# Borda/pyImSegm

Hardware: NVIDIA H100
Metric: megapixels/sec end-to-end SLIC+features+GC (pipe_color2d_slic_features_model_graphcut) (higher is better)
Workload: dtype f64

## Files before the change

include/imsegm_b200.h:

```cpp
#ifndef IMSEGM_B200_H
#define IMSEGM_B200_H

#include <stddef.h>
#include <stdint.h>

#ifdef __cplusplus
extern "C" {
#endif

typedef void* isb_stream_t;

enum isb_status {
    ISB_OK = 0,
    ISB_ERR_ARG = -1,
    ISB_ERR_CUDA = -2,
    ISB_ERR_CAPACITY = -3,
    ISB_ERR_UNSUPPORTED = -4
};

enum isb_dtype { ISB_U8 = 0, ISB_U16 = 1, ISB_F32 = 2, ISB_F64 = 3, ISB_I8 = 4, ISB_I16 = 5, ISB_I32 = 6, ISB_U32 = 7, ISB_I64 = 8, ISB_BOOL = 9 };

const char* isb_last_error(void);
int isb_abi_version(void);
long long isb_launch_count(void);
int isb_note_graph_replay(long long n_kernels);
int isb_profile_enable(int on);
int isb_profile_stage_count(void);
const char* isb_profile_stage_name(int id);
int isb_profile_collect(double* ms_out , long long* count_out );


int isb_slic_prepare(const void* img, int dtype, int H, int W, int C, const double* w_half, int radius, double ratio,
                     int rescale, double* lab_planar, double* minmax_out , isb_stream_t stream);

int isb_image_minmax(const void* img, int dtype, long long n, double* minmax_out , isb_stream_t stream);

size_t isb_slic_kmeans_workspace_bytes(int H, int W, int n_seeds, int step_y, int step_x);

int isb_slic_kmeans(const double* lab_planar, int H, int W, const double* seeds_yx, int n_seeds, int step_y, int step_x,
                    double step, int max_iter, int slic_zero, int32_t* labels, double* centroids, void* ws, size_t ws_bytes,
                    isb_stream_t stream);

int isb_slic_set_tile_cap(int cap);
long long isb_slic_full_scan_tiles(void);

typedef struct isb_slic_band {
    int32_t slab_rows, width;
    int32_t image_rows, y_off;
    int32_t own_lo, own_hi;
    int32_t halo;
    int32_t n_seeds, step_y, step_x, slic_zero;
    double step;
    const double* lab_slab;
    size_t plane_stride;
    const double* seeds_yx;
    int32_t* labels_slab;
    void* ws; size_t ws_bytes;
} isb_slic_band_t;
int isb_slic_band_begin(const isb_slic_band_t* band, isb_stream_t stream);
int isb_slic_band_assign(const isb_slic_band_t* band, isb_stream_t stream);
int isb_slic_band_update(const isb_slic_band_t* band, int64_t* xchg, isb_stream_t stream);
int isb_slic_band_import(const isb_slic_band_t* band, const int64_t* xchg, uint64_t* maxdc_xchg ,
                         isb_stream_t stream);
int isb_slic_band_finalize(const isb_slic_band_t* band, const uint64_t* maxdc_xchg, isb_stream_t stream);

size_t isb_connectivity_workspace_bytes(int H, int W);


int isb_enforce_connectivity(const int32_t* labels, int H, int W, int min_size, int max_size, int32_t* out,
                             int32_t* n_labels_out, void* ws, size_t ws_bytes, isb_stream_t stream);

int isb_slic3d_prepare(const void* vol, int dtype, int D, int H, int W, const double* w_z, int r_z, const double* w_y, int r_y,
                       const double* w_x, int r_x, double ratio, double* tmp, double* out, isb_stream_t stream);
size_t isb_slic3d_kmeans_workspace_bytes(int D, int H, int W, int n_seeds);
int isb_slic3d_kmeans(const double* vol_scaled, int D, int H, int W, const double* seeds_zyx, int n_seeds, int step_z, int step_y,
                      int step_x, double step, const double* spacing_host, int max_iter, int32_t* labels, void* ws, size_t ws_bytes,
                      isb_stream_t stream);
size_t isb_connectivity3d_workspace_bytes(int D, int H, int W, int max_size);
int isb_enforce_connectivity3d(const int32_t* labels, int D, int H, int W, int min_size, int max_size, int32_t* out,
                               int32_t* n_labels_out, void* ws, size_t ws_bytes, isb_stream_t stream);


size_t isb_segment_stats_workspace_bytes(int nb);
int isb_segment_stats_2d(const void* img, int dtype, const int32_t* seg, int H, int W, int nb, int flags, double* feat,
                         int ld, int col0, double* centres, int32_t* counts, void* ws, size_t ws_bytes, isb_stream_t stream);

int isb_segment_stats_accumulate(const void* img, int dtype, const int32_t* seg, int H, int W, int y_off, int nb, double* acc,
                                 int64_t* iacc, isb_stream_t stream);
int isb_segment_stats_deviation(const void* img, int dtype, const int32_t* seg, int H, int W, int nb, const double* acc,
                                const int64_t* iacc, float* meanf_scratch , double* var, isb_stream_t stream);
int isb_segment_stats_finish(int nb, int flags, const double* acc, const double* var, const int64_t* iacc, double* feat, int ld,
                             int col0, double* centres, int32_t* counts, isb_stream_t stream);

size_t isb_gray_stats_workspace_bytes(int nb);
int isb_gray_stats(const void* img, int dtype, const int32_t* seg, long long n, int nb, int flags, double* feat, int ld, int col0,
                   void* ws, size_t ws_bytes, isb_stream_t stream);

int isb_label_hist_2d(const int16_t* segm_select, const int16_t* struc_elem, int H, int W, int nb_labels, uint32_t* hist,
                      isb_stream_t stream);

int isb_region_label_hist(const int32_t* slic, const int32_t* annot, int H, int W, int nb_slic, int nb_annot, uint32_t* hist,
                          isb_stream_t stream);

int isb_filter_response_2d(const double* img, int n_slices, int H, int W, const double* kernels, int n_kernels, int kh, int kw,
                           double* out, isb_stream_t stream);

int isb_gaussian_filter_2d(const double* img, int n_slices, int H, int W, const double* w_half, int radius, double* tmp, double* out,
                           isb_stream_t stream);

enum isb_color_space { ISB_COLOR_HSV = 0, ISB_COLOR_LUV = 1, ISB_COLOR_LAB = 2, ISB_COLOR_HED = 3, ISB_COLOR_XYZ = 4 };
int isb_color_convert(const void* img, int dtype, long long n_px, int space, double* out, isb_stream_t stream);
int isb_gradient_sum_2d(const void* img, int dtype, int H, int W, int channels, void* out, isb_stream_t stream);
int isb_segment_median_2d(const void* img, int dtype, const int32_t* seg, int H, int W, int channels, int nb, double* feat, int ld,
                          int col0, void* ws, size_t ws_bytes, isb_stream_t stream);

int isb_lm_background(const void* img, int dtype, int H, int W, const double* w_half, int radius, const double* mix, double* planar,
                      double* tmp, double* smooth, isb_stream_t stream);
size_t isb_lm_battery_workspace_bytes(void);
int isb_lm_battery_response(const double* planar, int H, int W, const double* kernels, int n_kernels, int kh, int kw, double max_signal,
                            double* resp, double* out, void* ws, size_t ws_bytes, isb_stream_t stream);
int isb_lm_battery_partial(const double* planar, int H, int W, const double* kernels, int n_kernels, int kh, int kw, double max_signal,
                           int row_lo, int row_hi, double* resp, double* sumsq, void* ws, size_t ws_bytes, isb_stream_t stream);
int isb_lm_battery_scale(const double* resp, int H, int W, int row_lo, int row_hi, double max_signal, const double* sumsq, double* out,
                         isb_stream_t stream);

int isb_disc_label_hist(const int32_t* segm, const double* proba, int H, int W, const int32_t* positions, int n_pos,
                        const int32_t* diameters, int n_diam, const uint8_t* selem, int mh, int mw, int nb_labels, double* hist,
                        double* sizes, isb_stream_t stream);

int isb_ray_features_2d(const int8_t* seg_binary, int H, int W, const int32_t* positions, int n_pos, const float* sin_a,
                        const float* cos_a, int n_ang, int edge, float* out, isb_stream_t stream);


size_t isb_adjacency_workspace_bytes(int nb, int cap);
int isb_adjacency_edges(const int32_t* seg, int H, int W, int nb, int32_t* edges, int cap, int32_t* n_edges_out, void* ws,
                        size_t ws_bytes, isb_stream_t stream);

int isb_adjacency_edges_3d(const int32_t* seg, int D, int H, int W, int nb, int32_t* edges, int cap, int32_t* n_edges_out, void* ws,
                           size_t ws_bytes, isb_stream_t stream);
int isb_centroids_3d(const int32_t* seg, int D, int H, int W, int nb, double* centres, void* ws, size_t ws_bytes, isb_stream_t stream);

int isb_gc_energies(const double* proba, int N, const int32_t* n_nodes_dev , int K, const int32_t* edges, int E,
                    const int32_t* n_edges_dev,
                    const double* centres, int metric, int spatial, double edge_cost, const double* pairwise ,
                    double* unary, double* edge_w, int32_t* unary_i, int32_t* edge_wi, int32_t* smooth_i, void* ws,
                    size_t ws_bytes, isb_stream_t stream);
size_t isb_gc_energies_workspace_bytes(int N, int K, int E);

size_t isb_alpha_expansion_workspace_bytes(int N, int K, int E);
int isb_alpha_expansion(int N, const int32_t* n_nodes_dev , int K, int E, const int32_t* n_edges_dev,
                        const int32_t* edges, const int32_t* edge_wi,
                        const int32_t* unary_i, const int32_t* smooth_i, int n_iter, int32_t* labels, int64_t* energy_out,
                        int32_t* stats_out , void* ws, size_t ws_bytes,
                        isb_stream_t stream);

size_t isb_mixture_fit_workspace_bytes(int kind, int N, int D, int K, int n_init);
int isb_mixture_fit_params_len(int kind, int D, int K);
int isb_mixture_fit_predict(int kind, const double* feat, int N, int D, int ld, const int32_t* n_dev, int K, int n_init, int max_iter,
                            double tol, double reg_covar, int use_scaler, unsigned long long seed, const int32_t* init_labels, double* proba,
                            double* params_out, void* ws, size_t ws_bytes, isb_stream_t stream);
size_t isb_pca_workspace_bytes(int N, int D);
int isb_pca_params_len(int D);
int isb_pca_fit(const double* feat, int N, int D, int ld, const int32_t* n_dev, int use_scaler, double coef, int n_components,
                double* params_out, int32_t* n_components_out, void* ws, size_t ws_bytes, isb_stream_t stream);

size_t isb_class_transform_workspace_bytes(int N, int D_in, int has_pca);
int isb_class_transform(const double* feat, int N, int ld, const int32_t* n_dev, int D_in, const double* sc_mean, const double* sc_scale,
                        const double* pca_comp, const double* pca_mean, const double* pca_scale, int D_out, double* out, void* ws,
                        size_t ws_bytes, isb_stream_t stream);
size_t isb_mixture_predict_workspace_bytes(int N, int D, int K);
int isb_mixture_predict_proba(const double* x, int N, const int32_t* n_dev, int D, int K, const double* prec_chol, const double* bvec,
                              const double* log_const, double* proba, void* ws, size_t ws_bytes, isb_stream_t stream);
size_t isb_forest_predict_workspace_bytes(int N, int n_trees);
int isb_forest_predict_proba(const double* x, int N, const int32_t* n_dev, int D, int n_trees, const int32_t* roots, const int32_t* feature,
                             const double* threshold, const int32_t* left, const int32_t* right, int n_nodes, const double* value, int K,
                             int average, double* proba, void* ws, size_t ws_bytes, isb_stream_t stream);
size_t isb_knn_predict_workspace_bytes(int N, int N_t, int k);
int isb_knn_predict_proba(const double* x, int N, const int32_t* n_dev, int D, const double* fit_x, int N_t, const int32_t* y, int k, int K,
                          int weights, double* proba, void* ws, size_t ws_bytes, isb_stream_t stream);
size_t isb_linear_predict_workspace_bytes(int N, int n_coef);
int isb_linear_predict_proba(const double* x, int N, const int32_t* n_dev, int D, const double* coef, const double* intercept, int n_coef,
                             double* proba, void* ws, size_t ws_bytes, isb_stream_t stream);

size_t isb_lm_workspace_bytes(int H, int W, int nb, int n_batt);
int isb_lm_texture(const void* img, int dtype, const int32_t* seg, int H, int W, int nb, const double* bg_weights, int bg_radius,
                   const double* chmix_host, const float* w_tc, int NP, int orient, int n_batt, int flags,
                   double* feat, int ld, int col0, void* ws, size_t ws_bytes, isb_stream_t stream);
size_t isb_lm_acc_doubles(int nb, int n_batt);
int isb_lm_texture_accumulate(const void* img, int dtype, const int32_t* seg, int slab_rows, int W, int y_first, int y_end, int nb,
                              const double* bg_weights, int bg_radius, const double* chmix_host, const float* w_tc, int NP, int orient,
                              int n_batt, double* acc, int32_t* counts, void* ws, size_t ws_bytes, isb_stream_t stream);
int isb_lm_texture_finish(int nb, int n_batt, int flags, const double* acc, const int32_t* counts, double* feat, int ld, int col0,
                          isb_stream_t stream);

int isb_wgmma_selftest(const float* A, const float* B, int N, int K, int variant, float* D, isb_stream_t stream);

size_t isb_segment_median_workspace_bytes(long long n_px, int nb);
int isb_segment_median(const void* img, int dtype, const int32_t* seg, long long n_px, int channels, int nb, double* out, void* ws,
                       size_t ws_bytes, isb_stream_t stream);


int isb_ellipse_ransac(int T, const int32_t* trial_centre, const int32_t* samp_off, const int32_t* samp_idx, const double* params_in,
                       int C, const double* pts, const int32_t* pt_off, double thr, const double* sp_pts, const int32_t* sp_lab,
                       const double* lab_term, int N, int32_t* ok, double* params_out, int32_t* n_inl, double* crit,
                       double* resid_out, const long long* resid_off, isb_stream_t stream);
int isb_ellipse_overlap(const int32_t* segm, int H, int W, int n_labels, const int32_t* bbox_host, const double* geom_host,
                        uint8_t* mask, unsigned long long* counts, isb_stream_t stream);
int isb_binary_morph_footprint(const uint8_t* in, int H, int W, const int32_t* offsets, int n_offsets, int op, uint8_t* out,
                               isb_stream_t stream);


int isb_label_boundary_map(const int32_t* seg, int H, int W, uint8_t* out, isb_stream_t stream);
int isb_label_contour_map(const int32_t* seg, int H, int W, int32_t label, int include_boundary, uint8_t* out, isb_stream_t stream);
size_t isb_edt_workspace_bytes(int H, int W);
int isb_edt_2d(const uint8_t* sites, int H, int W, double* dist, void* ws, size_t ws_bytes, isb_stream_t stream);
size_t isb_edt_index_workspace_bytes(int H, int W);
int isb_edt_2d_indices(const uint8_t* sites, int H, int W, int32_t* index, void* ws, size_t ws_bytes, isb_stream_t stream);
size_t isb_mask_compact_workspace_bytes(int H, int W);
int isb_mask_compact_count(const uint8_t* mask, int H, int W, void* ws, size_t ws_bytes, long long* total, isb_stream_t stream);
int isb_mask_compact_write(const uint8_t* mask, int H, int W, const double* values, const void* ws, size_t ws_bytes, int64_t* points,
                           double* values_out, isb_stream_t stream);
int isb_relabel_gather(const int32_t* seg, long long npx, const int32_t* lut, int n_lut, int32_t* out, isb_stream_t stream);


int isb_color_hist(const uint8_t* img, long long n_px, int channels, int accumulate, unsigned long long* hist, isb_stream_t stream);
size_t isb_color_hist_workspace_bytes(void);
int isb_color_hist_compact_count(const unsigned long long* hist, void* ws, size_t ws_bytes, long long* total, isb_stream_t stream);
int isb_color_hist_compact_write(const unsigned long long* hist, const void* ws, size_t ws_bytes, int32_t* colors, int64_t* counts,
                                 isb_stream_t stream);
int isb_palette_map(const void* img, int dtype, long long n_px, int channels, const void* palette, int n_colors, int mode,
                    const int64_t* values, int64_t* labels, uint8_t* matched, unsigned long long* unmatched, isb_stream_t stream);
int isb_palette_gather(const int64_t* labels, long long n_px, const int64_t* keys, int n_colors, const void* table, int row_bytes,
                       void* out, unsigned long long* missing, isb_stream_t stream);
int isb_gather_at_index(const void* src, int elem_bytes, const int32_t* index, long long n, void* out, isb_stream_t stream);


size_t isb_contingency_workspace_bytes(int dtype_true, int dtype_pred);
int isb_contingency_count(const void* y_true, int dtype_true, const void* y_pred, int dtype_pred, long long n, const int64_t* drop, int n_drop,
                          void* ws, size_t ws_bytes, long long* info, isb_stream_t stream);
int isb_contingency_write(const void* y_true, int dtype_true, const void* y_pred, int dtype_pred, long long n, const int64_t* drop, int n_drop,
                          const long long* info, void* ws, size_t ws_bytes, int64_t* values_true, int64_t* values_pred, int64_t* counts,
                          isb_stream_t stream);

size_t isb_kmeans_workspace_bytes(int n, int k, int D);
int isb_kmeans_lloyd(const double* X, int n, int D, int k, int max_iter, int sweeps, double tol, double* centres, int32_t* labels, int32_t* status,
                     double* sums, int32_t* counts, double* inertia, void* ws, size_t ws_bytes, isb_stream_t stream);
int isb_kmeans_nearest(const double* X, int n, int D, const double* centres, int k, int32_t* nearest, void* ws, size_t ws_bytes,
                       isb_stream_t stream);

size_t isb_forest_fit_workspace_bytes(int n, int D, int T, int K, int max_features);
int isb_forest_fit(const float* x, int n, int D, const int32_t* y, int K, const int32_t* counts, int T, const uint64_t* seeds, int max_features,
                   int min_samples_split, int min_samples_leaf, int max_depth, double min_impurity_decrease, int cap, int32_t* left, int32_t* right,
                   int32_t* feature, double* threshold, double* impurity, int32_t* n_node_samples, double* weighted_n_node_samples,
                   uint8_t* missing_go_to_left, int32_t* class_counts, int32_t* node_count, int* n_levels , void* ws, size_t ws_bytes,
                   isb_stream_t stream);

size_t isb_forest_fit_groups_workspace_bytes(int n, int Dmax, int G, int T, int K, int max_features_max);
int isb_forest_fit_groups(const float* x, int n, int Dmax, int G, const int32_t* D , const int32_t* max_features ,
                          const int32_t* min_samples_split , const int32_t* min_samples_leaf , const int32_t* y, int K,
                          const int32_t* counts, int T, const int32_t* tree_group , const uint64_t* seeds, int max_depth,
                          double min_impurity_decrease, int cap, int32_t* left, int32_t* right, int32_t* feature, double* threshold,
                          double* impurity, int32_t* n_node_samples, double* weighted_n_node_samples, uint8_t* missing_go_to_left,
                          int32_t* class_counts, int32_t* node_count, int* n_levels , void* ws, size_t ws_bytes, isb_stream_t stream);

size_t isb_extra_trees_fit_workspace_bytes(int n, int D, int T, int K, int max_features);
int isb_extra_trees_fit(const float* x, int n, int D, const int32_t* y, int K, const int32_t* counts, int T, const uint32_t* rand_r_state,
                        int max_features, int min_samples_split, int min_samples_leaf, int max_depth, double min_impurity_decrease,
                        int small_rows, int cap, int32_t* left, int32_t* right, int32_t* feature, double* threshold, double* impurity,
                        int32_t* n_node_samples, double* weighted_n_node_samples, uint8_t* missing_go_to_left, int32_t* class_counts,
                        int32_t* node_count, void* ws, size_t ws_bytes, isb_stream_t stream);

int isb_fill_i32(int32_t* dst, long long n, int32_t value, isb_stream_t stream);

int isb_combine(void* dst, const void* src, long long n, int op, isb_stream_t stream);

int isb_gather(const int32_t* seg, long long npx, const int32_t* lut_i, const double* lut_p, int K, int32_t* out_i,
               double* out_p, isb_stream_t stream);

#ifdef __cplusplus
}
#endif
#endif
```

pyimsegm_b200/_lib.py:

```python
import ctypes as C
import os

_HERE = os.path.dirname(os.path.abspath(__file__))
LIB_PATH = os.path.join(_HERE, 'libimsegm_b200.so')

_lib = None

ISB_OK, ISB_ERR_ARG, ISB_ERR_CUDA, ISB_ERR_CAPACITY, ISB_ERR_UNSUPPORTED = 0, -1, -2, -3, -4
DTYPE_CODES = {'uint8': 0, 'uint16': 1, 'float32': 2, 'float64': 3}

_vp, _i, _d, _sz, _ll = C.c_void_p, C.c_int, C.c_double, C.c_size_t, C.c_longlong



class SlicBand(C.Structure):
    _fields_ = [('slab_rows', C.c_int32), ('width', C.c_int32), ('image_rows', C.c_int32), ('y_off', C.c_int32),
                ('own_lo', C.c_int32), ('own_hi', C.c_int32), ('halo', C.c_int32),
                ('n_seeds', C.c_int32), ('step_y', C.c_int32), ('step_x', C.c_int32), ('slic_zero', C.c_int32),
                ('step', C.c_double), ('lab_slab', C.c_void_p), ('plane_stride', C.c_size_t), ('seeds_yx', C.c_void_p),
                ('labels_slab', C.c_void_p), ('ws', C.c_void_p), ('ws_bytes', C.c_size_t)]


_bp = C.POINTER(SlicBand)

SIGNATURES = {
    'isb_last_error': (C.c_char_p, []),
    'isb_abi_version': (_i, []),
    'isb_launch_count': (_ll, []),
    'isb_note_graph_replay': (_i, [_ll]),
    'isb_profile_enable': (_i, [_i]),
    'isb_profile_stage_count': (_i, []),
    'isb_profile_stage_name': (C.c_char_p, [_i]),
    'isb_profile_collect': (_i, [C.POINTER(_d), C.POINTER(_ll)]),
    'isb_slic_prepare': (_i, [_vp, _i, _i, _i, _i, C.POINTER(_d), _i, _d, _i, _vp, _vp, _vp]),
    'isb_image_minmax': (_i, [_vp, _i, _ll, _vp, _vp]),
    'isb_slic_band_begin': (_i, [_bp, _vp]),
    'isb_slic_band_assign': (_i, [_bp, _vp]),
    'isb_slic_band_update': (_i, [_bp, _vp, _vp]),
    'isb_slic_band_import': (_i, [_bp, _vp, _vp, _vp]),
    'isb_slic_band_finalize': (_i, [_bp, _vp, _vp]),
    'isb_segment_stats_accumulate': (_i, [_vp, _i, _vp, _i, _i, _i, _i, _vp, _vp, _vp]),
    'isb_segment_stats_deviation': (_i, [_vp, _i, _vp, _i, _i, _i, _vp, _vp, _vp, _vp, _vp]),
    'isb_segment_stats_finish': (_i, [_i, _i, _vp, _vp, _vp, _vp, _i, _i, _vp, _vp, _vp]),
    'isb_slic_kmeans_workspace_bytes': (_sz, [_i, _i, _i, _i, _i]),
    'isb_slic_kmeans': (_i, [_vp, _i, _i, _vp, _i, _i, _i, _d, _i, _i, _vp, _vp, _vp, _sz, _vp]),
    'isb_slic_set_tile_cap': (_i, [_i]),
    'isb_slic_full_scan_tiles': (_ll, []),
    'isb_slic3d_prepare': (_i, [_vp, _i, _i, _i, _i, _vp, _i, _vp, _i, _vp, _i, _d, _vp, _vp, _vp]),
    'isb_slic3d_kmeans_workspace_bytes': (_sz, [_i, _i, _i, _i]),
    'isb_slic3d_kmeans': (_i, [_vp, _i, _i, _i, _vp, _i, _i, _i, _i, _d, C.POINTER(_d), _i, _vp, _vp, _sz, _vp]),
    'isb_connectivity3d_workspace_bytes': (_sz, [_i, _i, _i, _i]),
    'isb_enforce_connectivity3d': (_i, [_vp, _i, _i, _i, _i, _i, _vp, _vp, _vp, _sz, _vp]),
    'isb_connectivity_workspace_bytes': (_sz, [_i, _i]),
    'isb_enforce_connectivity': (_i, [_vp, _i, _i, _i, _i, _vp, _vp, _vp, _sz, _vp]),
    'isb_segment_stats_workspace_bytes': (_sz, [_i]),
    'isb_segment_stats_2d': (_i, [_vp, _i, _vp, _i, _i, _i, _i, _vp, _i, _i, _vp, _vp, _vp, _sz, _vp]),
    'isb_adjacency_workspace_bytes': (_sz, [_i, _i]),
    'isb_adjacency_edges': (_i, [_vp, _i, _i, _i, _vp, _i, _vp, _vp, _sz, _vp]),
    'isb_adjacency_edges_3d': (_i, [_vp, _i, _i, _i, _i, _vp, _i, _vp, _vp, _sz, _vp]),
    'isb_centroids_3d': (_i, [_vp, _i, _i, _i, _i, _vp, _vp, _sz, _vp]),
    'isb_gc_energies_workspace_bytes': (_sz, [_i, _i, _i]),
    'isb_gc_energies': (_i, [_vp, _i, _vp, _i, _vp, _i, _vp, _vp, _i, _i, _d, _vp, _vp, _vp, _vp, _vp, _vp, _vp, _sz, _vp]),
    'isb_alpha_expansion_workspace_bytes': (_sz, [_i, _i, _i]),
    'isb_alpha_expansion': (_i, [_i, _vp, _i, _i, _vp, _vp, _vp, _vp, _vp, _i, _vp, _vp, _vp, _vp, _sz, _vp]),
    'isb_mixture_fit_workspace_bytes': (_sz, [_i, _i, _i, _i, _i]),
    'isb_mixture_fit_params_len': (_i, [_i, _i, _i]),
    'isb_mixture_fit_predict': (_i, [_i, _vp, _i, _i, _i, _vp, _i, _i, _i, _d, _d, _i, C.c_ulonglong, _vp, _vp, _vp, _vp, _sz, _vp]),
    'isb_pca_workspace_bytes': (_sz, [_i, _i]),
    'isb_pca_params_len': (_i, [_i]),
    'isb_pca_fit': (_i, [_vp, _i, _i, _i, _vp, _i, _d, _i, _vp, _vp, _vp, _sz, _vp]),
    'isb_class_transform_workspace_bytes': (_sz, [_i, _i, _i]),
    'isb_class_transform': (_i, [_vp, _i, _i, _vp, _i, _vp, _vp, _vp, _vp, _vp, _i, _vp, _vp, _sz, _vp]),
    'isb_mixture_predict_workspace_bytes': (_sz, [_i, _i, _i]),
    'isb_mixture_predict_proba': (_i, [_vp, _i, _vp, _i, _i, _vp, _vp, _vp, _vp, _vp, _sz, _vp]),
    'isb_forest_predict_workspace_bytes': (_sz, [_i, _i]),
    'isb_forest_predict_proba': (_i, [_vp, _i, _vp, _i, _i, _vp, _vp, _vp, _vp, _vp, _i, _vp, _i, _i, _vp, _vp, _sz, _vp]),
    'isb_knn_predict_workspace_bytes': (_sz, [_i, _i, _i]),
    'isb_knn_predict_proba': (_i, [_vp, _i, _vp, _i, _vp, _i, _vp, _i, _i, _i, _vp, _vp, _sz, _vp]),
    'isb_linear_predict_workspace_bytes': (_sz, [_i, _i]),
    'isb_linear_predict_proba': (_i, [_vp, _i, _vp, _i, _vp, _vp, _i, _vp, _vp, _sz, _vp]),
    'isb_lm_workspace_bytes': (_sz, [_i, _i, _i, _i]),
    'isb_lm_acc_doubles': (_sz, [_i, _i]),
    'isb_lm_texture_accumulate': (_i, [_vp, _i, _vp, _i, _i, _i, _i, _i, _vp, _i, C.POINTER(_d), _vp, _i, _i, _i, _vp, _vp, _vp, _sz, _vp]),
    'isb_lm_texture_finish': (_i, [_i, _i, _i, _vp, _vp, _vp, _i, _i, _vp]),
    'isb_lm_texture': (_i, [_vp, _i, _vp, _i, _i, _i, _vp, _i, C.POINTER(_d), _vp, _i, _i, _i, _i, _vp, _i, _i, _vp, _sz, _vp]),
    'isb_wgmma_selftest': (_i, [_vp, _vp, _i, _i, _i, _vp, _vp]),
    'isb_fill_i32': (_i, [_vp, _ll, _i, _vp]),
    'isb_combine': (_i, [_vp, _vp, _ll, _i, _vp]),
    'isb_gray_stats_workspace_bytes': (_sz, [_i]),
    'isb_gray_stats': (_i, [_vp, _i, _vp, _ll, _i, _i, _vp, _i, _i, _vp, _sz, _vp]),
    'isb_label_hist_2d': (_i, [_vp, _vp, _i, _i, _i, _vp, _vp]),
    'isb_ray_features_2d': (_i, [_vp, _i, _i, _vp, _i, _vp, _vp, _i, _i, _vp, _vp]),
    'isb_filter_response_2d': (_i, [_vp, _i, _i, _i, _vp, _i, _i, _i, _vp, _vp]),
    'isb_gaussian_filter_2d': (_i, [_vp, _i, _i, _i, _vp, _i, _vp, _vp, _vp]),
    'isb_disc_label_hist': (_i, [_vp, _vp, _i, _i, _vp, _i, _vp, _i, _vp, _i, _i, _i, _vp, _vp, _vp]),
    'isb_region_label_hist': (_i, [_vp, _vp, _i, _i, _i, _i, _vp, _vp]),
    'isb_gather': (_i, [_vp, _ll, _vp, _vp, _i, _vp, _vp, _vp]),
    'isb_segment_median_workspace_bytes': (_sz, [_ll, _i]),
    'isb_segment_median': (_i, [_vp, _i, _vp, _ll, _i, _i, _vp, _vp, _sz, _vp]),
    'isb_color_convert': (_i, [_vp, _i, _ll, _i, _vp, _vp]),
    'isb_gradient_sum_2d': (_i, [_vp, _i, _i, _i, _i, _vp, _vp]),
    'isb_segment_median_2d': (_i, [_vp, _i, _vp, _i, _i, _i, _i, _vp, _i, _i, _vp, _sz, _vp]),
    'isb_lm_background': (_i, [_vp, _i, _i, _i, _vp, _i, C.POINTER(_d), _vp, _vp, _vp, _vp]),
    'isb_lm_battery_workspace_bytes': (_sz, []),
    'isb_lm_battery_response': (_i, [_vp, _i, _i, _vp, _i, _i, _i, _d, _vp, _vp, _vp, _sz, _vp]),
    'isb_lm_battery_partial': (_i, [_vp, _i, _i, _vp, _i, _i, _i, _d, _i, _i, _vp, _vp, _vp, _sz, _vp]),
    'isb_lm_battery_scale': (_i, [_vp, _i, _i, _i, _i, _d, _vp, _vp, _vp]),
    'isb_ellipse_ransac': (_i, [_i, _vp, _vp, _vp, _vp, _i, _vp, _vp, _d, _vp, _vp, _vp, _i, _vp, _vp, _vp, _vp, _vp, _vp, _vp]),
    'isb_ellipse_overlap': (_i, [_vp, _i, _i, _i, C.POINTER(C.c_int32), C.POINTER(_d), _vp, _vp, _vp]),
    'isb_binary_morph_footprint': (_i, [_vp, _i, _i, _vp, _i, _i, _vp, _vp]),
    'isb_label_boundary_map': (_i, [_vp, _i, _i, _vp, _vp]),
    'isb_label_contour_map': (_i, [_vp, _i, _i, C.c_int32, _i, _vp, _vp]),
    'isb_edt_workspace_bytes': (_sz, [_i, _i]),
    'isb_edt_2d': (_i, [_vp, _i, _i, _vp, _vp, _sz, _vp]),
    'isb_mask_compact_workspace_bytes': (_sz, [_i, _i]),
    'isb_mask_compact_count': (_i, [_vp, _i, _i, _vp, _sz, _vp, _vp]),
    'isb_mask_compact_write': (_i, [_vp, _i, _i, _vp, _vp, _sz, _vp, _vp, _vp]),
    'isb_relabel_gather': (_i, [_vp, _ll, _vp, _i, _vp, _vp]),
    'isb_edt_index_workspace_bytes': (_sz, [_i, _i]),
    'isb_edt_2d_indices': (_i, [_vp, _i, _i, _vp, _vp, _sz, _vp]),
    'isb_color_hist': (_i, [_vp, _ll, _i, _i, _vp, _vp]),
    'isb_color_hist_workspace_bytes': (_sz, []),
    'isb_color_hist_compact_count': (_i, [_vp, _vp, _sz, _vp, _vp]),
    'isb_color_hist_compact_write': (_i, [_vp, _vp, _sz, _vp, _vp, _vp]),
    'isb_palette_map': (_i, [_vp, _i, _ll, _i, _vp, _i, _i, _vp, _vp, _vp, _vp, _vp]),
    'isb_palette_gather': (_i, [_vp, _ll, _vp, _i, _vp, _i, _vp, _vp, _vp]),
    'isb_gather_at_index': (_i, [_vp, _i, _vp, _ll, _vp, _vp]),
    'isb_contingency_workspace_bytes': (_sz, [_i, _i]),
    'isb_contingency_count': (_i, [_vp, _i, _vp, _i, _ll, _vp, _i, _vp, _sz, C.POINTER(_ll), _vp]),
    'isb_contingency_write': (_i, [_vp, _i, _vp, _i, _ll, _vp, _i, C.POINTER(_ll), _vp, _sz, _vp, _vp, _vp, _vp]),
    'isb_kmeans_workspace_bytes': (_sz, [_i, _i, _i]),
    'isb_kmeans_lloyd': (_i, [_vp, _i, _i, _i, _i, _i, _d, _vp, _vp, _vp, _vp, _vp, _vp, _vp, _sz, _vp]),
    'isb_kmeans_nearest': (_i, [_vp, _i, _i, _vp, _i, _vp, _vp, _sz, _vp]),
    'isb_forest_fit_workspace_bytes': (_sz, [_i, _i, _i, _i, _i]),
    'isb_forest_fit': (_i, [_vp, _i, _i, _vp, _i, _vp, _i, _vp, _i, _i, _i, _i, _d, _i, _vp, _vp, _vp, _vp, _vp, _vp, _vp, _vp, _vp, _vp,
                            C.POINTER(_i), _vp, _sz, _vp]),
    'isb_forest_fit_groups_workspace_bytes': (_sz, [_i, _i, _i, _i, _i, _i]),
    'isb_forest_fit_groups': (_i, [_vp, _i, _i, _i, _vp, _vp, _vp, _vp, _vp, _i, _vp, _i, _vp, _vp, _i, _d, _i, _vp, _vp, _vp, _vp, _vp, _vp,
                                   _vp, _vp, _vp, _vp, C.POINTER(_i), _vp, _sz, _vp]),
    'isb_extra_trees_fit_workspace_bytes': (_sz, [_i, _i, _i, _i, _i]),
    'isb_extra_trees_fit': (_i, [_vp, _i, _i, _vp, _i, _vp, _i, _vp, _i, _i, _i, _i, _d, _i, _i, _vp, _vp, _vp, _vp, _vp, _vp, _vp, _vp, _vp,
                                 _vp, _vp, _sz, _vp]),
}


class NativeLibraryError(RuntimeError):
    pass


def lib():
    global _lib
    if _lib is None:
        if not os.path.isfile(LIB_PATH):
            raise NativeLibraryError(
                'pyimsegm_b200: %s is missing -- build it with `python -m pyimsegm_b200.build` '
                '(there is no CPU fallback)' % LIB_PATH)
        handle = C.CDLL(LIB_PATH)
        for name, (res, args) in SIGNATURES.items():
            fn = getattr(handle, name)
            fn.restype = res
            fn.argtypes = args
        _lib = handle
    return _lib


def check(status):
    if status != ISB_OK:
        msg = lib().isb_last_error().decode(errors='replace')
        if status == ISB_ERR_ARG:
            raise ValueError('imsegm_b200: ' + msg)
        if status == ISB_ERR_UNSUPPORTED:
            raise NotImplementedError('imsegm_b200: ' + msg)
        raise RuntimeError('imsegm_b200 (status %d): %s' % (status, msg))


def require_cuda():
    import torch
    if not torch.cuda.is_available():
        raise NativeLibraryError('pyimsegm_b200 needs a CUDA device (H100 / sm_90a); there is no CPU fallback')
    return torch


def dtype_code(dtype):
    return DTYPE_CODES[str(dtype).replace('torch.', '')]


def ptr(t):
    return None if t is None else C.c_void_p(t.data_ptr())


def stream_ptr():
    import torch
    return C.c_void_p(torch.cuda.current_stream().cuda_stream)
```

pyimsegm_b200/csrc/slic_prepare.cu:

```cuda
#include "common.cuh"

namespace {

struct GaussW { double w[9]; };

__device__ __forceinline__ double dadd(double a, double b) { return __dadd_rn(a, b); }
__device__ __forceinline__ double dsub(double a, double b) { return __dsub_rn(a, b); }
__device__ __forceinline__ double dmul(double a, double b) { return __dmul_rn(a, b); }
__device__ __forceinline__ double ddiv(double a, double b) { return __ddiv_rn(a, b); }

__device__ __forceinline__ double det_cbrt(double x)
{
    unsigned long long u = 0x553EF00000000000ull - (unsigned long long)__double_as_longlong(x) / 3ull;
    double y = __longlong_as_double((long long)u);
#pragma unroll
    for (int i = 0; i < 4; ++i) {
        const double y2 = dmul(y, y);
        const double y3 = dmul(y2, y);
        const double t = dmul(x, y3);
        const double w = dsub(4.0, t);
        y = dmul(dmul(y, w), 1.0 / 3.0);
    }
    const double y2 = dmul(y, y);
    double c = dmul(x, y2);
    const double c3 = dmul(dmul(c, c), c);
    c = dsub(c, dmul(dmul(dsub(c3, x), y2), 1.0 / 3.0));
    return c;
}

__device__ __forceinline__ double det_root5(double x)
{
    unsigned long long u = 0x4CB8A99999999800ull - (unsigned long long)__double_as_longlong(x) / 5ull;
    double y = __longlong_as_double((long long)u);
#pragma unroll
    for (int i = 0; i < 4; ++i) {
        const double y2 = dmul(y, y);
        const double y4 = dmul(y2, y2);
        const double y5 = dmul(y4, y);
        const double t = dmul(x, y5);
        const double w = dsub(6.0, t);
        y = dmul(dmul(y, w), 0.2);
    }
    const double y2 = dmul(y, y);
    const double y4 = dmul(y2, y2);
    double r = dmul(x, y4);
    const double r2 = dmul(r, r);
    const double r5 = dmul(dmul(r2, r2), r);
    r = dsub(r, dmul(dmul(dsub(r5, x), y4), 0.2));
    return r;
}

__device__ __forceinline__ double det_pow24(double t)
{
    double r = det_root5(t);
    return dmul(dmul(t, t), dmul(r, r));
}

__device__ __forceinline__ void rgb2lab_px(double r, double g, double b, double& L, double& A, double& B)
{
    double c[3] = { r, g, b };
#pragma unroll
    for (int i = 0; i < 3; ++i) {
        if (c[i] > 0.04045) c[i] = det_pow24(ddiv(dadd(c[i], 0.055), 1.055));
        else c[i] = ddiv(c[i], 12.92);
    }
    double X = dadd(dadd(dmul(c[0], 0.412453), dmul(c[1], 0.357580)), dmul(c[2], 0.180423));
    double Y = dadd(dadd(dmul(c[0], 0.212671), dmul(c[1], 0.715160)), dmul(c[2], 0.072169));
    double Z = dadd(dadd(dmul(c[0], 0.019334), dmul(c[1], 0.119193)), dmul(c[2], 0.950227));
    double f[3] = { ddiv(X, 0.95047), ddiv(Y, 1.0), ddiv(Z, 1.08883) };
#pragma unroll
    for (int i = 0; i < 3; ++i) {
        if (f[i] > 0.008856) f[i] = det_cbrt(f[i]);
        else f[i] = dadd(dmul(7.787, f[i]), ddiv(16.0, 116.0));
    }
    L = dsub(dmul(116.0, f[1]), 16.0);
    A = dmul(500.0, dsub(f[0], f[1]));
    B = dmul(200.0, dsub(f[1], f[2]));
}

__global__ void k_minmax(const void* img, int dtype, size_t n, unsigned long long* mm)
{
    double lo = 1.0 / 0.0, hi = -1.0 / 0.0;
    for (size_t i = (size_t)blockIdx.x * blockDim.x + threadIdx.x; i < n; i += (size_t)gridDim.x * blockDim.x) {
        double v = load_as_f64(img, dtype, i);
        lo = fmin(lo, v);
        hi = fmax(hi, v);
    }
#pragma unroll
    for (int o = 16; o > 0; o >>= 1) {
        lo = fmin(lo, __shfl_xor_sync(0xffffffffu, lo, o));
        hi = fmax(hi, __shfl_xor_sync(0xffffffffu, hi, o));
    }
    __shared__ double slo[32], shi[32];
    int w = threadIdx.x >> 5, l = threadIdx.x & 31;
    if (l == 0) { slo[w] = lo; shi[w] = hi; }
    __syncthreads();
    if (w == 0) {
        int nw = blockDim.x >> 5;
        lo = l < nw ? slo[l] : 1.0 / 0.0;
        hi = l < nw ? shi[l] : -1.0 / 0.0;
#pragma unroll
        for (int o = 16; o > 0; o >>= 1) {
            lo = fmin(lo, __shfl_xor_sync(0xffffffffu, lo, o));
            hi = fmax(hi, __shfl_xor_sync(0xffffffffu, hi, o));
        }
        if (l == 0) {
            atomicMin(&mm[0], f64_ordered(lo));
            atomicMax(&mm[1], f64_ordered(hi));
        }
    }
}

__global__ void k_minmax_decode(const unsigned long long* mm, double* out)
{
    out[0] = f64_unordered(mm[0]);
    out[1] = f64_unordered(mm[1]);
}

constexpr int TX = 128, SH = 64, KR = 8, NT = 256;

template <int R>
struct BlurShape {
    static constexpr int IW = TX + 2 * R;
    static constexpr int RING = 2 * R + KR;
    static constexpr size_t smem = sizeof(double) * 3 * ((size_t)RING * IW + (size_t)KR * IW) + sizeof(int) * IW;
};

template <int R>
__global__ void __launch_bounds__(NT, 2) k_blur_lab(const void* __restrict__ img, int dtype, int H, int W, int C,
                                                    const double* __restrict__ minmax, int rescale, GaussW gw, double ratio,
                                                    double* __restrict__ out)
{
    using S = BlurShape<R>;
    constexpr int IW = S::IW, RING = S::RING;
    extern __shared__ double smem[];
    double* s_in = smem;
    double* s_v = smem + 3 * RING * IW;
    int* s_gx = (int*)(s_v + 3 * KR * IW);
    const int x0 = blockIdx.x * TX, y0 = blockIdx.y * SH;
    const int y_end = min(y0 + SH, H);
    const double mn = minmax[0], mx = minmax[1];
    const bool do_rescale = rescale && (mn != 0.0 || mx != 1.0);
    const double span = dsub(mx, mn);
    const size_t HW = (size_t)H * W;

    for (int ix = threadIdx.x; ix < IW; ix += NT) s_gx[ix] = reflect_index(x0 + ix - R, W);
    __syncthreads();

    auto prep = [&](double v) {
        if (do_rescale) v = ddiv(dsub(v, mn), span);
        if (R > 0) {
            double t = dmul(v, gw.w[0]);
#pragma unroll
            for (int j = R; j >= 1; --j) t = dadd(t, dmul(dadd(v, v), gw.w[j]));
            v = t;
        }
        return v;
    };

    int slot0 = 0;
    for (int cy = y0; cy < y_end; cy += KR) {
        const int first = cy == y0;
        const int lo = first ? 0 : cy - y0 + 2 * R, nrow = first ? RING : KR;
        for (int i = threadIdx.x; i < nrow * IW; i += NT) {
            const int row = i / IW, ix = i - row * IW;
            const int ir = lo + row;
            const int gy = reflect_index(y0 - R + ir, H);
            const size_t base = ((size_t)gy * W + s_gx[ix]) * C;
            double* dst = s_in + (ir % RING) * IW + ix;
            if (C == 3) {
#pragma unroll
                for (int c = 0; c < 3; ++c) dst[c * RING * IW] = prep(load_as_f64(img, dtype, base + c));
            } else {
                const double v = prep(load_as_f64(img, dtype, base));
#pragma unroll
                for (int c = 0; c < 3; ++c) dst[c * RING * IW] = v;
            }
        }
        __syncthreads();
        for (int i = threadIdx.x; i < 3 * IW; i += NT) {
            const int c = i / IW, ix = i - c * IW;
            const double* col = s_in + c * RING * IW + ix;
            double w[RING];
#pragma unroll
            for (int k = 0; k < RING; ++k) {
                int s = slot0 + k;
                if (s >= RING) s -= RING;
                w[k] = col[s * IW];
            }
            double* dst = s_v + c * KR * IW + ix;
#pragma unroll
            for (int k = 0; k < KR; ++k) {
                double t = w[k + R];
                if (R > 0) {
                    t = dmul(w[k + R], gw.w[0]);
#pragma unroll
                    for (int j = R; j >= 1; --j) t = dadd(t, dmul(dadd(w[k + R - j], w[k + R + j]), gw.w[j]));
                }
                dst[k * IW] = t;
            }
        }
        __syncthreads();
        for (int i = threadIdx.x; i < KR * TX; i += NT) {
            const int ty = i / TX, tx = i - ty * TX;
            const int gy = cy + ty, gx = x0 + tx;
            if (gy >= y_end || gx >= W) continue;
            double v[3];
#pragma unroll
            for (int c = 0; c < 3; ++c) {
                const double* row = s_v + (c * KR + ty) * IW + tx + R;
                double t = row[0];
                if (R > 0) {
                    t = dmul(row[0], gw.w[0]);
#pragma unroll
                    for (int j = R; j >= 1; --j) t = dadd(t, dmul(dadd(row[-j], row[j]), gw.w[j]));
                }
                v[c] = t;
            }
            double L, A, B;
            rgb2lab_px(v[0], v[1], v[2], L, A, B);
            const size_t p = (size_t)gy * W + gx;
            out[p] = dmul(L, ratio);
            out[HW + p] = dmul(A, ratio);
            out[2 * HW + p] = dmul(B, ratio);
        }
        slot0 += KR;
        if (slot0 >= RING) slot0 -= RING;
    }
}

template <int R>
static int blur_lab_launch(const void* img, int dtype, int H, int W, int C, const double* minmax, int rescale, const GaussW& gw,
                           double ratio, double* out, cudaStream_t st)
{
    const size_t smem = BlurShape<R>::smem;
    if (smem > 48 * 1024) ISB_CUDA_CHECK(cudaFuncSetAttribute(k_blur_lab<R>, cudaFuncAttributeMaxDynamicSharedMemorySize, (int)smem));
    dim3 grid((W + TX - 1) / TX, (H + SH - 1) / SH);
    k_blur_lab<R><<<grid, NT, smem, st>>>(img, dtype, H, W, C, minmax, rescale, gw, ratio, out);
    ISB_LAUNCH_CHECK();
    return ISB_OK;
}

static int minmax_launch(const void* img, int dtype, size_t n, double* minmax_out, cudaStream_t st)
{
    unsigned long long* mm = (unsigned long long*)(minmax_out + 2);
    ISB_CUDA_CHECK(cudaMemsetAsync(mm, 0xFF, sizeof(unsigned long long), st));
    ISB_CUDA_CHECK(cudaMemsetAsync(mm + 1, 0x00, sizeof(unsigned long long), st));
    int blocks = (int)((n + 256 * 8 - 1) / (256 * 8));
    if (blocks > 132 * 8) blocks = 132 * 8;
    if (blocks < 1) blocks = 1;
    k_minmax<<<blocks, 256, 0, st>>>(img, dtype, n, mm);
    ISB_LAUNCH_CHECK();
    k_minmax_decode<<<1, 1, 0, st>>>(mm, minmax_out);
    ISB_LAUNCH_CHECK();
    return ISB_OK;
}

}

extern "C" int isb_image_minmax(const void* img, int dtype, long long n, double* minmax_out, isb_stream_t stream)
{
    ISB_REQUIRE(img && minmax_out && n > 0, "null pointer or empty image");
    ISB_REQUIRE(dtype >= ISB_U8 && dtype <= ISB_F64, "bad dtype");
    return minmax_launch(img, dtype, (size_t)n, minmax_out, (cudaStream_t)stream);
}

extern "C" int isb_slic_prepare(const void* img, int dtype, int H, int W, int C, const double* w_half, int radius, double ratio,
                                int rescale, double* lab_planar, double* minmax_out, isb_stream_t stream)
{
    ISB_REQUIRE(img && lab_planar && minmax_out, "null pointer");
    ISB_REQUIRE(H > 0 && W > 0 && (C == 1 || C == 3), "bad image shape (C must be 1 or 3)");
    ISB_REQUIRE(dtype >= ISB_U8 && dtype <= ISB_F64, "bad dtype");
    ISB_REQUIRE(radius >= 0 && radius <= 8 && (radius == 0 || w_half), "gaussian radius must be in [0,8]");
    cudaStream_t st = (cudaStream_t)stream;
    ProfScope prof(ISB_PROF_PREPARE, st);
    if (rescale != 2)
        if (int rc = minmax_launch(img, dtype, (size_t)H * W * C, minmax_out, st)) return rc;
    GaussW gw;
    for (int i = 0; i < 9; ++i) gw.w[i] = (i <= radius && w_half) ? w_half[i] : 0.0;
    switch (radius) {
        case 0: return blur_lab_launch<0>(img, dtype, H, W, C, minmax_out, rescale, gw, ratio, lab_planar, st);
        case 1: return blur_lab_launch<1>(img, dtype, H, W, C, minmax_out, rescale, gw, ratio, lab_planar, st);
        case 2: return blur_lab_launch<2>(img, dtype, H, W, C, minmax_out, rescale, gw, ratio, lab_planar, st);
        case 3: return blur_lab_launch<3>(img, dtype, H, W, C, minmax_out, rescale, gw, ratio, lab_planar, st);
        case 4: return blur_lab_launch<4>(img, dtype, H, W, C, minmax_out, rescale, gw, ratio, lab_planar, st);
        case 5: return blur_lab_launch<5>(img, dtype, H, W, C, minmax_out, rescale, gw, ratio, lab_planar, st);
        case 6: return blur_lab_launch<6>(img, dtype, H, W, C, minmax_out, rescale, gw, ratio, lab_planar, st);
        case 7: return blur_lab_launch<7>(img, dtype, H, W, C, minmax_out, rescale, gw, ratio, lab_planar, st);
        default: return blur_lab_launch<8>(img, dtype, H, W, C, minmax_out, rescale, gw, ratio, lab_planar, st);
    }
}
```

Baseline: 1557.

## Speed up SLIC prepare: reciprocal division, cp.async blur loads, vectorized minmax

```diff
diff --git a/include/imsegm_b200.h b/include/imsegm_b200.h
--- a/include/imsegm_b200.h
+++ b/include/imsegm_b200.h
@@ -195,6 +195,8 @@
 
 int isb_wgmma_selftest(const float* A, const float* B, int N, int K, int variant, float* D, isb_stream_t stream);
 
+int isb_div_recip_check(const double* a, long long n, double b, int steps, unsigned long long* res, isb_stream_t stream);
+
 size_t isb_segment_median_workspace_bytes(long long n_px, int nb);
 int isb_segment_median(const void* img, int dtype, const int32_t* seg, long long n_px, int channels, int nb, double* out, void* ws,
                        size_t ws_bytes, isb_stream_t stream);
diff --git a/pyimsegm_b200/_lib.py b/pyimsegm_b200/_lib.py
--- a/pyimsegm_b200/_lib.py
+++ b/pyimsegm_b200/_lib.py
@@ -85,6 +85,7 @@
     'isb_lm_texture_finish': (_i, [_i, _i, _i, _vp, _vp, _vp, _i, _i, _vp]),
     'isb_lm_texture': (_i, [_vp, _i, _vp, _i, _i, _i, _vp, _i, C.POINTER(_d), _vp, _i, _i, _i, _i, _vp, _i, _i, _vp, _sz, _vp]),
     'isb_wgmma_selftest': (_i, [_vp, _vp, _i, _i, _i, _vp, _vp]),
+    'isb_div_recip_check': (_i, [_vp, _ll, _d, _i, _vp, _vp]),
     'isb_fill_i32': (_i, [_vp, _ll, _i, _vp]),
     'isb_combine': (_i, [_vp, _vp, _ll, _i, _vp]),
     'isb_gray_stats_workspace_bytes': (_sz, [_i]),
diff --git a/pyimsegm_b200/csrc/slic_prepare.cu b/pyimsegm_b200/csrc/slic_prepare.cu
--- a/pyimsegm_b200/csrc/slic_prepare.cu
+++ b/pyimsegm_b200/csrc/slic_prepare.cu
@@ -1,13 +1,49 @@
 #include "common.cuh"
+#include <string.h>
 
 namespace {
 
 struct GaussW { double w[9]; };
+
+template <typename T>
+__device__ __forceinline__ void cp_async(void* smem, const T* gmem)
+{
+    const unsigned dst = (unsigned)__cvta_generic_to_shared(smem);
+    asm volatile("cp.async.ca.shared.global [%0], [%1], %2;" ::"r"(dst), "l"(gmem), "n"(sizeof(T)));
+}
+__device__ __forceinline__ void cp_async_commit() { asm volatile("cp.async.commit_group;"); }
+__device__ __forceinline__ void cp_async_wait_all() { asm volatile("cp.async.wait_group 0;" ::: "memory"); }
 
 __device__ __forceinline__ double dadd(double a, double b) { return __dadd_rn(a, b); }
 __device__ __forceinline__ double dsub(double a, double b) { return __dsub_rn(a, b); }
 __device__ __forceinline__ double dmul(double a, double b) { return __dmul_rn(a, b); }
 __device__ __forceinline__ double ddiv(double a, double b) { return __ddiv_rn(a, b); }
+
+struct Recip {
+    double b, y;
+    bool two;
+};
+
+__device__ __forceinline__ Recip recip_of(double b)
+{
+    const double y = __ddiv_rn(1.0, b);
+    return Recip{ b, y, !(fabs(__fma_rn(y, b, -1.0)) <= 0x1p-54) };
+}
+
+__device__ __forceinline__ bool div_fast_range(double a)
+{
+    const long long bits = __double_as_longlong(a);
+    return bits == 0 || ((unsigned)(bits >> 52) & 0x7ffu) - 523u <= 1000u;
+}
+
+__device__ __forceinline__ double div_recip(double a, const Recip& d, bool& slow)
+{
+    double q = dmul(a, d.y);
+    q = __fma_rn(__fma_rn(-q, d.b, a), d.y, q);
+    if (d.two) q = __fma_rn(__fma_rn(-q, d.b, a), d.y, q);
+    slow |= !div_fast_range(a);
+    return q;
+}
 
 __device__ __forceinline__ double det_cbrt(double x)
 {
@@ -67,57 +103,119 @@
     double X = dadd(dadd(dmul(c[0], 0.412453), dmul(c[1], 0.357580)), dmul(c[2], 0.180423));
     double Y = dadd(dadd(dmul(c[0], 0.212671), dmul(c[1], 0.715160)), dmul(c[2], 0.072169));
     double Z = dadd(dadd(dmul(c[0], 0.019334), dmul(c[1], 0.119193)), dmul(c[2], 0.950227));
-    double f[3] = { ddiv(X, 0.95047), ddiv(Y, 1.0), ddiv(Z, 1.08883) };
+    double f[3] = { ddiv(X, 0.95047), Y, ddiv(Z, 1.08883) };
 #pragma unroll
     for (int i = 0; i < 3; ++i) {
         if (f[i] > 0.008856) f[i] = det_cbrt(f[i]);
-        else f[i] = dadd(dmul(7.787, f[i]), ddiv(16.0, 116.0));
+        else f[i] = dadd(dmul(7.787, f[i]), 16.0 / 116.0);
     }
     L = dsub(dmul(116.0, f[1]), 16.0);
     A = dmul(500.0, dsub(f[0], f[1]));
     B = dmul(200.0, dsub(f[1], f[2]));
 }
 
-__global__ void k_minmax(const void* img, int dtype, size_t n, unsigned long long* mm)
-{
+__device__ __forceinline__ void rgb2lab_warp(double r, double g, double b, double& L, double& A, double& B, bool& slow)
+{
+    constexpr Recip d_lin{ 12.92, 1.0 / 12.92, true }, d_gam{ 1.055, 1.0 / 1.055, false };
+    constexpr Recip d_xn{ 0.95047, 1.0 / 0.95047, false }, d_zn{ 1.08883, 1.0 / 1.08883, false };
+    const double v[3] = { r, g, b };
+    bool bright[3], s_gam[3] = { false, false, false }, s_lin[3] = { false, false, false };
+    double gam[3] = { 0.0, 0.0, 0.0 }, lin[3] = { 0.0, 0.0, 0.0 };
+#pragma unroll
+    for (int i = 0; i < 3; ++i) bright[i] = v[i] > 0.04045;
+    if (__any_sync(0xffffffffu, bright[0] || bright[1] || bright[2])) {
+#pragma unroll
+        for (int i = 0; i < 3; ++i) gam[i] = det_pow24(div_recip(dadd(v[i], 0.055), d_gam, s_gam[i]));
+    }
+    if (__any_sync(0xffffffffu, !(bright[0] && bright[1] && bright[2]))) {
+#pragma unroll
+        for (int i = 0; i < 3; ++i) lin[i] = div_recip(v[i], d_lin, s_lin[i]);
+    }
+    double c[3];
+#pragma unroll
+    for (int i = 0; i < 3; ++i) {
+        c[i] = bright[i] ? gam[i] : lin[i];
+        slow |= bright[i] ? s_gam[i] : s_lin[i];
+    }
+    const double X = dadd(dadd(dmul(c[0], 0.412453), dmul(c[1], 0.357580)), dmul(c[2], 0.180423));
+    const double Y = dadd(dadd(dmul(c[0], 0.212671), dmul(c[1], 0.715160)), dmul(c[2], 0.072169));
+    const double Z = dadd(dadd(dmul(c[0], 0.019334), dmul(c[1], 0.119193)), dmul(c[2], 0.950227));
+    double f[3] = { div_recip(X, d_xn, slow), Y, div_recip(Z, d_zn, slow) };
+#pragma unroll
+    for (int i = 0; i < 3; ++i) {
+        const double cube = det_cbrt(f[i]);
+        const double lin = dadd(dmul(7.787, f[i]), 16.0 / 116.0);
+        f[i] = f[i] > 0.008856 ? cube : lin;
+    }
+    L = dsub(dmul(116.0, f[1]), 16.0);
+    A = dmul(500.0, dsub(f[0], f[1]));
+    B = dmul(200.0, dsub(f[1], f[2]));
+}
+
+constexpr int MM_NT = 256, MM_UNROLL = 4;
+
+template <typename T>
+__global__ void __launch_bounds__(MM_NT) k_minmax(const T* __restrict__ img, size_t n, unsigned long long* out)
+{
+    constexpr int VEC = 16 / sizeof(T);
     double lo = 1.0 / 0.0, hi = -1.0 / 0.0;
-    for (size_t i = (size_t)blockIdx.x * blockDim.x + threadIdx.x; i < n; i += (size_t)gridDim.x * blockDim.x) {
-        double v = load_as_f64(img, dtype, i);
-        lo = fmin(lo, v);
-        hi = fmax(hi, v);
-    }
+    auto take = [&](T x) {
+        lo = fmin(lo, (double)x);
+        hi = fmax(hi, (double)x);
+    };
+    const size_t tid = (size_t)blockIdx.x * MM_NT + threadIdx.x, nthr = (size_t)gridDim.x * MM_NT;
+    size_t head = (16 - ((uintptr_t)img & 15)) / sizeof(T) % VEC;
+    if (head > n) head = n;
+    const size_t nv = (n - head) / VEC;
+    const uint4* v = (const uint4*)(img + head);
+    if (tid < head) take(img[tid]);
+    size_t i = tid;
+    for (; i + (MM_UNROLL - 1) * nthr < nv; i += MM_UNROLL * nthr) {
+        uint4 x[MM_UNROLL];
+#pragma unroll
+        for (int u = 0; u < MM_UNROLL; ++u) x[u] = __ldg(v + (nv - 1 - (i + u * nthr)));
+#pragma unroll
+        for (int u = 0; u < MM_UNROLL; ++u) {
+            const T* e = (const T*)&x[u];
+#pragma unroll
+            for (int k = 0; k < VEC; ++k) take(e[k]);
+        }
+    }
+    for (; i < nv; i += nthr) {
+        const uint4 x = __ldg(v + (nv - 1 - i));
+        const T* e = (const T*)&x;
+#pragma unroll
+        for (int k = 0; k < VEC; ++k) take(e[k]);
+    }
+    for (size_t j = head + nv * VEC + tid; j < n; j += nthr) take(img[j]);
 #pragma unroll
     for (int o = 16; o > 0; o >>= 1) {
         lo = fmin(lo, __shfl_xor_sync(0xffffffffu, lo, o));
         hi = fmax(hi, __shfl_xor_sync(0xffffffffu, hi, o));
     }
-    __shared__ double slo[32], shi[32];
-    int w = threadIdx.x >> 5, l = threadIdx.x & 31;
+    __shared__ double slo[MM_NT / 32], shi[MM_NT / 32];
+    const int w = threadIdx.x >> 5, l = threadIdx.x & 31;
     if (l == 0) { slo[w] = lo; shi[w] = hi; }
     __syncthreads();
-    if (w == 0) {
-        int nw = blockDim.x >> 5;
-        lo = l < nw ? slo[l] : 1.0 / 0.0;
-        hi = l < nw ? shi[l] : -1.0 / 0.0;
-#pragma unroll
-        for (int o = 16; o > 0; o >>= 1) {
-            lo = fmin(lo, __shfl_xor_sync(0xffffffffu, lo, o));
-            hi = fmax(hi, __shfl_xor_sync(0xffffffffu, hi, o));
-        }
-        if (l == 0) {
-            atomicMin(&mm[0], f64_ordered(lo));
-            atomicMax(&mm[1], f64_ordered(hi));
-        }
-    }
-}
-
-__global__ void k_minmax_decode(const unsigned long long* mm, double* out)
-{
-    out[0] = f64_unordered(mm[0]);
-    out[1] = f64_unordered(mm[1]);
+    if (threadIdx.x == 0) {
+#pragma unroll
+        for (int k = 1; k < MM_NT / 32; ++k) {
+            lo = fmin(lo, slo[k]);
+            hi = fmax(hi, shi[k]);
+        }
+        atomicMax(&out[2], ~f64_ordered(lo));
+        atomicMax(&out[3], f64_ordered(hi));
+        __threadfence();
+        if (atomicAdd(&out[0], 1ull) == gridDim.x - 1) {
+            __threadfence();
+            out[0] = (unsigned long long)__double_as_longlong(f64_unordered(~atomicAdd(&out[2], 0ull)));
+            out[1] = (unsigned long long)__double_as_longlong(f64_unordered(atomicAdd(&out[3], 0ull)));
+        }
+    }
 }
 
 constexpr int TX = 128, SH = 64, KR = 8, NT = 256;
+static_assert(KR * TX % NT == 0, "every lane of stage 3 runs the same number of pixels");
 
 template <int R>
 struct BlurShape {
@@ -142,13 +240,20 @@
     const double mn = minmax[0], mx = minmax[1];
     const bool do_rescale = rescale && (mn != 0.0 || mx != 1.0);
     const double span = dsub(mx, mn);
+    const bool span_fast = (((unsigned)__double2hiint(span)) >> 20) - 523u <= 1000u;
+    const Recip rspan = recip_of(span_fast ? span : 1.0);
     const size_t HW = (size_t)H * W;
 
     for (int ix = threadIdx.x; ix < IW; ix += NT) s_gx[ix] = reflect_index(x0 + ix - R, W);
     __syncthreads();
 
     auto prep = [&](double v) {
-        if (do_rescale) v = ddiv(dsub(v, mn), span);
+        if (do_rescale) {
+            const double a = dsub(v, mn);
+            bool slow = !span_fast;
+            v = div_recip(a, rspan, slow);
+            if (slow) v = ddiv(a, span);
+        }
         if (R > 0) {
             double t = dmul(v, gw.w[0]);
 #pragma unroll
@@ -158,25 +263,43 @@
         return v;
     };
 
-    int slot0 = 0;
-    for (int cy = y0; cy < y_end; cy += KR) {
-        const int first = cy == y0;
-        const int lo = first ? 0 : cy - y0 + 2 * R, nrow = first ? RING : KR;
+    auto fetch = [&](int lo, int nrow) {
         for (int i = threadIdx.x; i < nrow * IW; i += NT) {
             const int row = i / IW, ix = i - row * IW;
             const int ir = lo + row;
             const int gy = reflect_index(y0 - R + ir, H);
             const size_t base = ((size_t)gy * W + s_gx[ix]) * C;
             double* dst = s_in + (ir % RING) * IW + ix;
+            for (int c = 0; c < C; ++c) {
+                if (dtype == ISB_F64) cp_async(dst + c * RING * IW, (const double*)img + base + c);
+                else if (dtype == ISB_F32) cp_async(dst + c * RING * IW, (const float*)img + base + c);
+                else dst[c * RING * IW] = load_as_f64(img, dtype, base + c);
+            }
+        }
+        cp_async_commit();
+    };
+    auto finish = [&](int lo, int nrow) {
+        cp_async_wait_all();
+        for (int i = threadIdx.x; i < nrow * IW; i += NT) {
+            const int row = i / IW, ix = i - row * IW;
+            double* dst = s_in + ((lo + row) % RING) * IW + ix;
+            auto raw = [&](int c) { return dtype == ISB_F32 ? (double)*(const float*)(dst + c * RING * IW) : dst[c * RING * IW]; };
             if (C == 3) {
 #pragma unroll
-                for (int c = 0; c < 3; ++c) dst[c * RING * IW] = prep(load_as_f64(img, dtype, base + c));
+                for (int c = 0; c < 3; ++c) dst[c * RING * IW] = prep(raw(c));
             } else {
-                const double v = prep(load_as_f64(img, dtype, base));
+                const double v = prep(raw(0));
 #pragma unroll
                 for (int c = 0; c < 3; ++c) dst[c * RING * IW] = v;
             }
         }
+    };
+
+    int slot0 = 0;
+    fetch(0, RING);
+    for (int cy = y0; cy < y_end; cy += KR) {
+        const int first = cy == y0;
+        finish(first ? 0 : cy - y0 + 2 * R, first ? RING : KR);
         __syncthreads();
         for (int i = threadIdx.x; i < 3 * IW; i += NT) {
             const int c = i / IW, ix = i - c * IW;
@@ -201,10 +324,10 @@
             }
         }
         __syncthreads();
+        if (cy + KR < y_end) fetch(cy + KR - y0 + 2 * R, KR);
         for (int i = threadIdx.x; i < KR * TX; i += NT) {
             const int ty = i / TX, tx = i - ty * TX;
             const int gy = cy + ty, gx = x0 + tx;
-            if (gy >= y_end || gx >= W) continue;
             double v[3];
 #pragma unroll
             for (int c = 0; c < 3; ++c) {
@@ -218,7 +341,10 @@
                 v[c] = t;
             }
             double L, A, B;
-            rgb2lab_px(v[0], v[1], v[2], L, A, B);
+            bool slow = false;
+            rgb2lab_warp(v[0], v[1], v[2], L, A, B, slow);
+            if (gy >= y_end || gx >= W) continue;
+            if (slow) rgb2lab_px(v[0], v[1], v[2], L, A, B);
             const size_t p = (size_t)gy * W + gx;
             out[p] = dmul(L, ratio);
             out[HW + p] = dmul(A, ratio);
@@ -241,21 +367,65 @@
     return ISB_OK;
 }
 
-static int minmax_launch(const void* img, int dtype, size_t n, double* minmax_out, cudaStream_t st)
-{
-    unsigned long long* mm = (unsigned long long*)(minmax_out + 2);
-    ISB_CUDA_CHECK(cudaMemsetAsync(mm, 0xFF, sizeof(unsigned long long), st));
-    ISB_CUDA_CHECK(cudaMemsetAsync(mm + 1, 0x00, sizeof(unsigned long long), st));
-    int blocks = (int)((n + 256 * 8 - 1) / (256 * 8));
-    if (blocks > 132 * 8) blocks = 132 * 8;
-    if (blocks < 1) blocks = 1;
-    k_minmax<<<blocks, 256, 0, st>>>(img, dtype, n, mm);
-    ISB_LAUNCH_CHECK();
-    k_minmax_decode<<<1, 1, 0, st>>>(mm, minmax_out);
+template <typename T>
+static int minmax_launch_t(const void* img, size_t n, unsigned long long* out, cudaStream_t st)
+{
+    const size_t per_cta = (size_t)MM_NT * MM_UNROLL * (16 / sizeof(T));
+    size_t blocks = (n + per_cta - 1) / per_cta;
+    if (blocks > 132 * 4) blocks = 132 * 4;
+    k_minmax<T><<<(unsigned)blocks, MM_NT, 0, st>>>((const T*)img, n, out);
     ISB_LAUNCH_CHECK();
     return ISB_OK;
 }
 
+static int minmax_launch(const void* img, int dtype, size_t n, double* minmax_out, cudaStream_t st)
+{
+    static const int elem[4] = { 1, 2, 4, 8 };
+    ISB_REQUIRE((uintptr_t)img % elem[dtype] == 0, "image not aligned to its element size");
+    unsigned long long* out = (unsigned long long*)minmax_out;
+    ISB_CUDA_CHECK(cudaMemsetAsync(out, 0, 4 * sizeof(unsigned long long), st));
+    switch (dtype) {
+        case ISB_U8: return minmax_launch_t<unsigned char>(img, n, out, st);
+        case ISB_U16: return minmax_launch_t<unsigned short>(img, n, out, st);
+        case ISB_F32: return minmax_launch_t<float>(img, n, out, st);
+        default: return minmax_launch_t<double>(img, n, out, st);
+    }
+}
+
+__global__ void k_div_recip_check(const double* __restrict__ a, size_t n, double b, int steps, unsigned long long* res)
+{
+    Recip d = recip_of(b);
+    if (steps) d.two = steps == 2;
+    if (blockIdx.x == 0 && threadIdx.x == 0) res[3] = recip_of(b).two;
+    unsigned long long fast = 0;
+    for (size_t i = (size_t)blockIdx.x * blockDim.x + threadIdx.x; i < n; i += (size_t)gridDim.x * blockDim.x) {
+        bool slow = false;
+        const double q = div_recip(a[i], d, slow);
+        if (slow) continue;
+        ++fast;
+        if (__double_as_longlong(q) != __double_as_longlong(__ddiv_rn(a[i], b))) {
+            atomicAdd(&res[0], 1ull);
+            atomicMin(&res[1], (unsigned long long)i);
+        }
+    }
+    atomicAdd(&res[2], fast);
+}
+
+}
+
+extern "C" int isb_div_recip_check(const double* a, long long n, double b, int steps, unsigned long long* res, isb_stream_t stream)
+{
+    ISB_REQUIRE(a && res && n > 0, "null pointer or empty operand list");
+    ISB_REQUIRE(steps >= 0 && steps <= 2, "steps must be 0, 1 or 2");
+    unsigned long long bits;
+    memcpy(&bits, &b, sizeof bits);
+    ISB_REQUIRE((unsigned)(bits >> 52) - 523u <= 1000u, "divisor must be positive with an exponent in [-500, 500]");
+    cudaStream_t st = (cudaStream_t)stream;
+    ISB_CUDA_CHECK(cudaMemsetAsync(res, 0, 4 * sizeof(unsigned long long), st));
+    ISB_CUDA_CHECK(cudaMemsetAsync(res + 1, 0xFF, sizeof(unsigned long long), st));
+    k_div_recip_check<<<132 * 8, 256, 0, st>>>(a, (size_t)n, b, steps, res);
+    ISB_LAUNCH_CHECK();
+    return ISB_OK;
 }
 
 extern "C" int isb_image_minmax(const void* img, int dtype, long long n, double* minmax_out, isb_stream_t stream)
@@ -272,6 +442,8 @@
     ISB_REQUIRE(H > 0 && W > 0 && (C == 1 || C == 3), "bad image shape (C must be 1 or 3)");
     ISB_REQUIRE(dtype >= ISB_U8 && dtype <= ISB_F64, "bad dtype");
     ISB_REQUIRE(radius >= 0 && radius <= 8 && (radius == 0 || w_half), "gaussian radius must be in [0,8]");
+    static const int elem[4] = { 1, 2, 4, 8 };
+    ISB_REQUIRE((uintptr_t)img % elem[dtype] == 0, "image not aligned to its element size");
     cudaStream_t st = (cudaStream_t)stream;
     ProfScope prof(ISB_PROF_PREPARE, st);
     if (rescale != 2)
```

After: 1593 (median of 6 runs). 1.02x the previous value.
